# FeggieBoss/raytracing-course

Measured on AMD Instinct MI355X. Metric: Mray/s (closest-hit queries/s), dragon stand-in 1080p/256 spp, RAY_DEPTH 6, higher is better.
Workload: dtype f32

## Files before the change

### raytracing-course_amd/csrc/device/pt_query.h

```cpp
#pragma once
#include "pt_trace.h"

namespace pt {

#ifndef PT_AUXW
#define PT_AUXW 4
#endif

#define PT_LEAF_MARGIN 64.f

PT_HD float h16(uint32_t bits) { return (float)__builtin_bit_cast(_Float16, (uint16_t)(bits & 0xffffu)); }

PT_HD void aux_slab16(uint32_t w0, uint32_t w1, uint32_t w2, f3 inv, f3 oinv, float& tn, float& tf) {
    const float ax = fmaf(h16(w0), inv.x, -oinv.x), bx = fmaf(h16(w1 >> 16), inv.x, -oinv.x);
    const float ay = fmaf(h16(w0 >> 16), inv.y, -oinv.y), by = fmaf(h16(w2), inv.y, -oinv.y);
    const float az = fmaf(h16(w1), inv.z, -oinv.z), bz = fmaf(h16(w2 >> 16), inv.z, -oinv.z);
    tn = fmaxf(fmaxf(fminf(ax, bx), fminf(ay, by)), fminf(az, bz));
    tf = fminf(fminf(fmaxf(ax, bx), fmaxf(ay, by)), fmaxf(az, bz));
}

PT_HD bool aux_entry_hit(const F4& ea, const F4& eb, const Ray& ray, f3 inv, f3 oinv, float dlw) {
    if (signbit(dlw))
        return aux_box_par(h16(f2u(ea.x)), h16(f2u(ea.x) >> 16), h16(f2u(ea.y)), h16(f2u(ea.y) >> 16),
                           h16(f2u(ea.z)), h16(f2u(ea.z) >> 16), ray, inv, oinv);
    float tn, tf, un, uf;
    aux_slab16(f2u(ea.x), f2u(ea.y), f2u(ea.z), inv, oinv, tn, tf);
    aux_slab16(f2u(ea.w), f2u(eb.x), f2u(eb.y), inv, oinv, un, uf);
    const float mt = PT_LEAF_MARGIN * dlw;
    return tn <= tf && tf >= 0.f && (!(mt < INFINITY) || (un - mt <= uf + mt && uf + mt >= 0.f));
}

struct AuxSL { F4 a, b; };
#define PT_AUX_INTERNAL 0xffffffffu

enum : uint32_t { Q_AUX = 0u, Q_REPLAY = 1u, Q_DONE = 2u, Q_EXACT = 3u, Q_DECIDE = 4u };
enum : uint32_t { R_CAND = 0u, R_WALK_E = 1u, R_WALK_N = 2u };
#define PT_RKINDS 3u

#define PT_QPRIM_BYTES 64u
#define PT_QP_FULL 0x100u

PT_HD Prim qprim_expand(const F4& r0, const F4& r1, const F4& r2) {
    Prim P;
    const uint32_t type = f2u(r0.w);
    if (type == T_TRIANGLE) {
        P.p0 = F4{0.f, 0.f, 0.f, r0.w};
        P.p1 = F4{0.f, 0.f, 0.f, 1.f};
        P.p2 = F4{r0.x, r0.y, r0.z, 0.f};
        P.p3 = F4{r1.x, r1.y, r1.z, r2.x};
        P.p4 = F4{r2.y, r2.z, 0.f, 0.f};
    } else {
        P.p0 = F4{r1.x, r1.y, r1.z, r0.w};
        P.p1 = F4{r1.w, r2.x, r2.y, r2.z};
        P.p2 = F4{r0.x, r0.y, r0.z, 0.f};
        P.p3 = F4{0.f, 0.f, 0.f, 0.f};
        P.p4 = F4{0.f, 0.f, 0.f, 0.f};
    }
    return P;
}

#define PT_BUNDLE_BYTES 96u
#define PT_LEAFQ 0x80000000u

#ifndef PT_QHK
#define PT_QHK 6
#endif

struct Query {
    Ray ray;
    f3 inv;
    float P;
    uint32_t phase : 3;
    uint32_t walk : 2;
    uint32_t par : 1;
    uint32_t robust : 1;
    uint32_t known : 1;
    uint32_t overflow : 1;
    uint32_t sp : 7;
    uint32_t pos : 7;
    uint32_t len : 7;
    uint32_t nh : 4;
    uint32_t ne : 4;
    uint32_t cid : 10;
    uint32_t spare : 13;
    uint32_t node;
    uint32_t lb;
    uint32_t cand;
    float dl;
    union {
        struct {
            uint32_t lref, lcnt;
            uint32_t li;
            float lt;
            int lid;
            float lacc;
        };
        struct {
            uint32_t off;
            uint32_t e[4];
            uint32_t astar;
            float bound;
            float t1c, mc;
        };
    };
    uint32_t hidx[PT_QHK];
    float ht[PT_QHK];
    int hid[PT_QHK];
    float hacc[PT_QHK];
    float bt;
    float res_t;
    int res_id;
};
static_assert(PT_QHK < 16, "nh and ne are 4-bit fields");
#define PT_QUERY_SP_MAX 127u

struct QCounts {
    uint32_t nodes, aux, ptests, planes;
#ifdef PT_QDIAG
    uint32_t cands, passes, steps, rc_acc, rc_rej, rc_walk;
#endif
};

struct PlanesGlobal {
    const SceneView& S;
    PT_HD Prim operator()(uint32_t k, uint32_t& pi) const { pi = S.planes[k]; return S.prims[pi]; }
};
template <class PL>
PT_HD void q_planes_e(const SceneView& S, const PL& pl, const Ray& ray, float& P, int& pid) {
    P = PT_INF;
    pid = -1;
    for (uint32_t k = 0; k < S.n_planes; ++k) {
        uint32_t pi;
        const Prim pr = pl(k, pi);
        Hit h;
        bool ok;
        if (f2u(pr.p1.x) == 0u && f2u(pr.p1.y) == 0u && f2u(pr.p1.z) == 0u && f2u(pr.p1.w) == 0x3f800000u) {
            Ray lr;
            lr.o = ray.o + -1.f * mk3(pr.p0.x, pr.p0.y, pr.p0.z);
            lr.d = ray.d;
            ok = isect_plane(lr, mk3(pr.p2.x, pr.p2.y, pr.p2.z), h);
        } else {
            ok = plane_intersect(pr, ray, h);
        }
        if (ok && h.t < P) { P = h.t; pid = (int)pi; }
    }
}
PT_HD void q_planes(const SceneView& S, const Ray& ray, float& P, int& pid) { q_planes_e(S, PlanesGlobal{S}, ray, P, pid); }

PT_HD F4 q_prep(const SceneView& S, const Ray& ray) {
    const float big = 3e38f;
    if (!(fabsf(ray.o.x) < big && fabsf(ray.o.y) < big && fabsf(ray.o.z) < big && fabsf(ray.d.x) < big &&
          fabsf(ray.d.y) < big && fabsf(ray.d.z) < big))
        return F4{0.f, 0.f, 0.f, __builtin_nanf("")};
    const bool par = !replay_ok_ray(ray);
    const float om = fmaxf(fmaxf(fabsf(ray.o.x), fabsf(ray.o.y)), fabsf(ray.o.z));
    const float dm = fminf(fminf(fabsf(ray.d.x), fabsf(ray.d.y)), fabsf(ray.d.z));
    const float dl = par ? -INFINITY : 0x1p-18f * (S.box_extent + om) / dm;
    return F4{1.f / ray.d.x, 1.f / ray.d.y, 1.f / ray.d.z, dl};
}

PT_HD void q_init_pre(const Ray& ray, float P, int pid, F4 pre, Query& q) {
    q.ray = ray;
    q.res_id = pid;
    q.res_t = P;
    q.P = P;
    q.bt = PT_INF;
    q.nh = 0;
    q.ne = 0;
    q.lb = 0;
    q.overflow = 0;
    q.node = 0;
    q.sp = 0;
    q.li = 0;
#pragma unroll
    for (int i = 0; i < PT_QHK; ++i) q.hidx[i] = 0xffffffffu;
    q.inv = mk3(pre.x, pre.y, pre.z);
    q.par = signbit(pre.w) ? 1u : 0u;
    q.dl = fabsf(pre.w);
    q.phase = pre.w != pre.w ? Q_EXACT : Q_AUX;
}

PT_HD void q_init(const SceneView& S, const Ray& ray, float P, int pid, Query& q) {
    q_init_pre(ray, P, pid, q_prep(S, ray), q);
}

template <class T>
PT_HD T q_sel(const T (&a)[PT_QHK], uint32_t k, T dflt) {
    T v = dflt;
#pragma unroll
    for (int i = 0; i < PT_QHK; ++i)
        if ((uint32_t)i == k) v = a[i];
    return v;
}

PT_HD bool q_add_hit(Query& q, uint32_t c, float t, int id, float acc) {
    if (q.ne == PT_QHK) return false;
#pragma unroll
    for (int k = 0; k < PT_QHK; ++k) {
        const bool sw = q.hidx[k] > c;
        const uint32_t xi = q.hidx[k];
        const float xt = q.ht[k];
        const int xd = q.hid[k];
        const float xa = q.hacc[k];
        if (sw) {
            q.hidx[k] = c; q.ht[k] = t; q.hid[k] = id; q.hacc[k] = acc;
            c = xi; t = xt; id = xd; acc = xa;
        }
    }
    if (c != 0xffffffffu) q.overflow = 1u;
    else q.nh = q.nh + 1u;
    return true;
}

PT_HD void q_pass_done(Query& q) {
    if (q.overflow) {
        if (q.ne == PT_QHK) {
            q.phase = Q_EXACT;
            return;
        }
        q.overflow = 0;
        q.node = 0;
        q.sp = 0;
        q.li = 0;
        q.phase = Q_AUX;
        return;
    }
    q.phase = Q_DONE;
}

PT_HD void q_record_entered(Query& q) {
    const float t = q_sel(q.ht, q.ne, PT_INF);
    const int id = q_sel(q.hid, q.ne, -1);
    if (t < q.bt) {
        q.bt = t;
        if (t < q.P) { q.res_t = t; q.res_id = id; }
    }
    q.ne = q.ne + 1u;
    q.lb = q.cand + 1u;
}

PT_HD void q_next_decision(Query& q) { q.phase = Q_DECIDE; }

PT_HD void q_entered(Query& q) {
    q_record_entered(q);
    q_next_decision(q);
}

PT_HD void q_decide(Query& q) {
#pragma unroll 1
    while (q.ne < q.nh) {
        q.cand = q_sel(q.hidx, q.ne, 0xffffffffu);
        if (!(fminf(q.P, q.bt) >= q_sel(q.hacc, q.ne, PT_INF))) {
            q.walk = R_CAND;
            q.phase = Q_REPLAY;
            return;
        }
        q_record_entered(q);
    }
    q_pass_done(q);
}

PT_HD void q_rejected(Query& q) {
#pragma unroll
    for (int k = 0; k + 1 < PT_QHK; ++k) {
        if ((uint32_t)k >= q.ne) {
            q.hidx[k] = q.hidx[k + 1];
            q.ht[k] = q.ht[k + 1];
            q.hid[k] = q.hid[k + 1];
            q.hacc[k] = q.hacc[k + 1];
        }
    }
    q.hidx[PT_QHK - 1] = 0xffffffffu;
    q.nh = q.nh - 1u;
    q.lb = q.cand + 1u;
    q_next_decision(q);
}

PT_HD float q_bound_between(const Query& q, uint32_t a, uint32_t r) {
    float m = q.P;
    bool any = false;
#pragma unroll
    for (int k = 0; k < PT_QHK; ++k) {
        if ((uint32_t)k < q.ne && q.hidx[k] > a && q.hidx[k] < r) {
            if (!any || q.ht[k] < m) m = q.ht[k];
            any = true;
        }
    }
    return m;
}

PT_HD float q_leaf_accept_t(const Query& q, const F4& na, const F4& nb) {
    const f3 c = mk3(na.x, na.y, na.z);
    const f3 s = mk3(na.w, nb.x, nb.y);
    const f3 o = q.ray.o + -1.f * c;
    const f3 nlo = -1.f * s - o, nhi = s - o;
    const float ax = nlo.x * q.inv.x, bx = nhi.x * q.inv.x;
    const float ay = nlo.y * q.inv.y, by = nhi.y * q.inv.y;
    const float az = nlo.z * q.inv.z, bz = nhi.z * q.inv.z;
    const float t1 = smax(smax(smin(ax, bx), smin(ay, by)), smin(az, bz));
    const float t2 = smin(smin(smax(ax, bx), smax(ay, by)), smax(az, bz));
    const float m = q.dl + (fabsf(t1) + fabsf(t2)) * 0x1p-18f;
    const bool robust = !q.par && t1 + m <= t2 - m && t2 - m >= 0.f;
    return robust ? t1 + m : INFINITY;
}

PT_HD uint32_t q_leaf_certain(Query& q, const Node& nd) {
    float lo = q.P, hi = q.P;
#pragma unroll
    for (int k = 0; k < PT_QHK; ++k)
        if ((uint32_t)k < q.ne) { lo = fminf(lo, q.ht[k]); hi = fmaxf(hi, q.ht[k]); }
    const f3 c = mk3(nd.a.x, nd.a.y, nd.a.z);
    const f3 s = mk3(nd.a.w, nd.b.x, nd.b.y);
    const f3 o = q.ray.o + -1.f * c;
    const f3 nlo = -1.f * s - o, nhi = s - o;
    const float ax = nlo.x * q.inv.x, bx = nhi.x * q.inv.x;
    const float ay = nlo.y * q.inv.y, by = nhi.y * q.inv.y;
    const float az = nlo.z * q.inv.z, bz = nhi.z * q.inv.z;
    const float t1 = smax(smax(smin(ax, bx), smin(ay, by)), smin(az, bz));
    const float t2 = smin(smin(smax(ax, bx), smax(ay, by)), smax(az, bz));
    const float m = q.dl + (fabsf(t1) + fabsf(t2)) * 0x1p-18f;
    q.t1c = t1;
    q.mc = m;
    q.robust = (!q.par && t1 + m <= t2 - m && t2 - m >= 0.f) ? 1u : 0u;
    if (q.robust && lo >= t1 + m) return 1u;
    uint32_t v = q.par ? 2u : enter_decide(t1, t2, hi);
    if (v == 2u) v = enter_exact(nd.a, nd.b, q.ray, hi) ? 1u : 0u;
    return v == 0u ? 0u : 2u;
}


PT_HD void q_addr(const SceneView& S, const Query& q, uint32_t off[8]) {
    uint32_t b0, b1, b2;
    if (q.phase == Q_AUX) {
        if (!(q.node & PT_LEAFQ)) {
            const uint32_t b = S.o_aux + q.node * (uint32_t)(PT_AUXW * sizeof(AuxSL));
#pragma unroll
            for (int k = 0; k < 8; ++k) off[k] = b + 16u * (uint32_t)k;
            return;
        }
        if (q.li == 0u) {
            b0 = S.o_bundle + PT_BUNDLE_BYTES * (q.node & 0x7fffffffu);
#pragma unroll
            for (int k = 0; k < 8; ++k) off[k] = b0 + 16u * (uint32_t)(k < 6 ? k : 5);
            return;
        }
        if (q.li & 0x80000000u) {
            b0 = S.o_prim + 80u * (q.lref + (q.li & 0x7fffffffu));
#pragma unroll
            for (int k = 0; k < 8; ++k) off[k] = b0 + 16u * (uint32_t)(k < 5 ? k : 4);
            return;
        }
        b0 = S.o_qprim + PT_QPRIM_BYTES * (q.lref + q.li);
#pragma unroll
        for (int k = 0; k < 8; ++k) off[k] = b0 + 16u * (uint32_t)(k < 4 ? k : 3);
        return;
    } else if (q.walk == R_CAND) {
        b0 = S.o_nodes + 32u * q.cand;
        b1 = b0 + 16u;
        b2 = S.o_ainfo + 16u * (q.cand >> 2);
    } else if (q.walk == R_WALK_E) {
        b0 = S.o_anc + 4u * (q.off + q.pos);
        b1 = b0;
        b2 = b0;
    } else {
#pragma unroll
        for (int j = 0; j < 4; ++j) {
            const uint32_t e = q.e[j] == 0xffffffffu ? 0u : q.e[j];
            off[2 * j] = S.o_nodes + 32u * e;
            off[2 * j + 1] = off[2 * j] + 16u;
        }
        return;
    }
    off[0] = b0; off[1] = b1; off[2] = b2;
#pragma unroll
    for (int k = 3; k < 8; ++k) off[k] = b0;
}

template <class Mem>
PT_HD void q_aux_next(Query& q, Mem& stk, uint32_t next) {
    if (next == 0xffffffffu && q.sp > 0u) next = stk.get(--q.sp);
    if (next != 0xffffffffu) {
        q.node = next;
        return;
    }
    q_next_decision(q);
}

#if defined(PT_QPROF) && defined(__HIP_DEVICE_COMPILE__)
#define PT_QPROF_DEV 1
#define QP_STAMP(i) do { uint64_t t_; asm volatile("s_memtime %0\n\ts_waitcnt lgkmcnt(0)" : "=s"(t_)::"memory"); qp[i] = (uint32_t)t_; } while (0)
#define QP_ARG , uint32_t* qp
#else
#define QP_STAMP(i) (void)0
#define QP_ARG
#endif
template <class Mem>
PT_HD void q_exec_aux(const SceneView& S, Query& q, QCounts& C, Mem& stk, const F4 r[8]) {
    C.aux++;
    const f3 oinv = mk3(q.ray.o.x * q.inv.x, q.ray.o.y * q.inv.y, q.ray.o.z * q.inv.z);
    const float mt = PT_LEAF_MARGIN * q.dl;
    const bool mwide = !(mt < INFINITY);
    bool hit[PT_AUXW];
#pragma unroll
    for (int k = 0; k < PT_AUXW; ++k) {
        const F4 ea = r[2 * k], eb = r[2 * k + 1];
        float tn, tf, un, uf;
        aux_slab16(f2u(ea.x), f2u(ea.y), f2u(ea.z), q.inv, oinv, tn, tf);
        aux_slab16(f2u(ea.w), f2u(eb.x), f2u(eb.y), q.inv, oinv, un, uf);
        hit[k] = tn <= tf && tf >= 0.f && (mwide || (un - mt <= uf + mt && uf + mt >= 0.f));
    }
    if (pt_any(q.par != 0u)) {
#pragma unroll
        for (int k = 0; k < PT_AUXW; ++k) {
            const F4 ea = r[2 * k];
            if (q.par)
                hit[k] = aux_box_par(h16(f2u(ea.x)), h16(f2u(ea.x) >> 16), h16(f2u(ea.y)), h16(f2u(ea.y) >> 16),
                                     h16(f2u(ea.z)), h16(f2u(ea.z) >> 16), q.ray, q.inv, oinv);
        }
    }
    uint32_t next = 0xffffffffu;
    const uint32_t hmax = q.hidx[PT_QHK - 1];
    uint32_t sp = q.sp;
    bool ovf = false;
#pragma unroll
    for (int k = 0; k < PT_AUXW; ++k) {
        const uint32_t code = f2u(r[2 * k + 1].w);
        const uint32_t rng = f2u(r[2 * k + 1].z);
        const bool h = hit[k] && code != 0xffffffffu;
        const bool isleaf = (code & 0x80000000u) != 0u;
        const uint32_t lidx = code & 0x7fffffffu;
        const bool above = isleaf ? lidx > hmax
                                  : (hmax != 0xffffffffu && ((rng & 0xffffu) << S.aux_rshift) > hmax);
        const bool fresh = isleaf ? lidx >= q.lb : ((rng >> 16) << S.aux_rshift) >= q.lb;
        ovf = ovf || (h && fresh && above);
        const bool take = h && fresh && !above;
        const uint32_t item = isleaf ? (PT_LEAFQ | rng) : code;
        const bool first = take && next == 0xffffffffu;
        const bool push = take && !first;
        next = first ? item : next;
        stk.setc(sp, item, push && sp < stk.cap);
        sp += push ? 1u : 0u;
    }
    if (ovf) q.overflow = 1u;
    if (sp > stk.cap) {
        q.phase = Q_EXACT;
        return;
    }
    q.sp = sp;
#ifdef PT_QDIAG
    if (next == 0xffffffffu && q.sp == 0u) C.passes++;
    if (q.sp > C.steps) C.steps = q.sp;
#endif
    q_aux_next(q, stk, next);
}

template <class Mem>
PT_HD void q_exec_kind(const SceneView& S, Query& q, QCounts& C, Mem& stk, const F4 r[8] QP_ARG) {
    if (q.phase == Q_AUX && !(q.node & PT_LEAFQ)) {
        QP_STAMP(0);
        q_exec_aux(S, q, C, stk, r);
        return;
    }
    if (q.phase == Q_AUX) {
        QP_STAMP(1);
        if (q.li == 0u) {
            q.cand = f2u(r[3].x);
            q.lref = f2u(r[3].y);
            q.lcnt = f2u(r[3].z);
            q.lt = PT_INF;
            q.lid = -1;
            q.lacc = q_leaf_accept_t(q, r[4], r[5]);
#ifdef PT_QDIAG
            C.cands++;
#endif
            if (q.lcnt == 0u) {
                q_aux_next(q, stk, 0xffffffffu);
                return;
            }
        }
        const bool full = (q.li & 0x80000000u) != 0u;
        const uint32_t cty = f2u(r[0].w);
        if (!full && (cty & PT_QP_FULL)) {
            q.li |= 0x80000000u;
            return;
        }
        Prim pr = qprim_expand(r[0], r[1], r[2]);
        if (full) { pr.p0 = r[0]; pr.p1 = r[1]; pr.p2 = r[2]; pr.p3 = r[3]; pr.p4 = r[4]; }
        const uint32_t ty = f2u(pr.p0.w);
        Ray lr = q.ray;
        if (full || cty != T_TRIANGLE) {
            const f3 pos = mk3(pr.p0.x, pr.p0.y, pr.p0.z);
            lr.o = q.ray.o + -1.f * pos;
            const bool ident = f2u(pr.p1.x) == 0u && f2u(pr.p1.y) == 0u && f2u(pr.p1.z) == 0u &&
                               f2u(pr.p1.w) == 0x3f800000u;
            if (!ident) {
                q4 qq;
                qq.x = pr.p1.x; qq.y = pr.p1.y; qq.z = pr.p1.z; qq.w = pr.p1.w;
                const q4 cq = conj(qq);
                lr.o = qrot(cq, lr.o);
                lr.d = qrot(cq, q.ray.d);
            }
        }
        const f3 pa = mk3(pr.p2.x, pr.p2.y, pr.p2.z);
        bool ok;
        float t = 0.f;
        uint32_t in;
        if (ty == T_TRIANGLE) {
            const f3 pb = mk3(pr.p3.x, pr.p3.y, pr.p3.z), pc = mk3(pr.p3.w, pr.p4.x, pr.p4.y);
            f3 n = mk3(r[1].w, r[2].w, q.li == 0u ? r[3].w : r[3].x);
            if (full) n = normalize(cross(pb - pa, pc - pa));
            Hit h;
            ok = isect_triangle_n(lr, pa, pb, pc, n, h);
            t = h.t;
        } else if (ty == T_BOX) {
            ok = slab(lr.o, lr.d, pa, t, in);
        } else {
            ok = ellipsoid_root(lr, pa, t, in);
        }
        const uint32_t li = q.li & 0x7fffffffu;
        C.ptests++;
        if (ok && t < q.lt) { q.lt = t; q.lid = (int)(q.lref + li); }
        q.li = li + 1u;
        if (q.li < q.lcnt) return;
        q.li = 0u;
        if (q.lid >= 0 && !q_add_hit(q, q.cand, q.lt, q.lid, q.lacc)) {
            q.phase = Q_EXACT;
            return;
        }
        q_aux_next(q, stk, 0xffffffffu);
        return;
    }
    if (q.walk == R_CAND) {
        QP_STAMP(2);
        Node nd;
        nd.a = r[0];
        nd.b = r[1];
        const uint32_t k4 = q.cand & 3u;
        const uint32_t info = f2u(k4 == 0u ? r[2].x : k4 == 1u ? r[2].y : k4 == 2u ? r[2].z : r[2].w);
        C.nodes++;
        const uint32_t v = q_leaf_certain(q, nd);
#ifdef PT_QDIAG
        if (v == 1u) C.rc_acc++; else if (v == 0u) C.rc_rej++; else C.rc_walk++;
#endif
        if (v == 1u) {
            q_entered(q);
            return;
        }
        if (v == 0u) {
            q_rejected(q);
            return;
        }
        q.off = info & 0x03ffffffu;
        q.len = info >> 26;
        q.pos = 0u;
        q.known = q.ne == 0u ? 1u : 0u;
        q.bound = q.P;
        q.astar = 0u;
        q.walk = R_WALK_E;
        return;
    }
    if (q.walk == R_WALK_E) {
        QP_STAMP(3);
        const uint32_t hlast = q_sel(q.hidx, q.ne - 1u, 0u);
        bool any = false, accept = false;
        const uint32_t ent[4] = {f2u(r[0].x), f2u(r[0].y), f2u(r[0].z), f2u(r[0].w)};
#pragma unroll
        for (int j = 0; j < 4; ++j) {
            uint32_t e = q.pos + (uint32_t)j < q.len ? ent[j] : 0xffffffffu;
            if (e != 0xffffffffu && !accept && !q.known) {
                if (e <= hlast) {
                    q.astar = e;
                    e = 0xffffffffu;
                } else {
                    q.bound = q_bound_between(q, q.astar, e);
                    q.known = 1u;
                    if (q.robust && q.bound >= q.t1c + q.mc) accept = true;
                }
            }
            if (accept) e = 0xffffffffu;
            q.e[j] = e;
            any = any || e != 0xffffffffu;
        }
        if (accept) {
            q_entered(q);
            return;
        }
        if (any) q.walk = R_WALK_N;
        else q.pos += 4u;
        return;
    }
    QP_STAMP(4);
    bool reject = false;
#pragma unroll
    for (int j = 0; j < 4; ++j) {
        if (q.e[j] == 0xffffffffu) continue;
        Node nd;
        nd.a = r[2 * j];
        nd.b = r[2 * j + 1];
        C.nodes++;
        if (!node_enter(nd, q.ray, q.inv, q.bound, q.par != 0u)) reject = true;
    }
    if (reject) {
        q_rejected(q);
        return;
    }
    q.pos += 4u;
    if (q.pos >= q.len) q_entered(q);
    else q.walk = R_WALK_E;
}

template <class Mem>
PT_HD void q_exec(const SceneView& S, Query& q, QCounts& C, Mem& stk, const F4 r[8] QP_ARG) {
#ifdef PT_QPROF_DEV
    q_exec_kind(S, q, C, stk, r, qp);
#else
    q_exec_kind(S, q, C, stk, r);
#endif
    if (q.phase == Q_DECIDE) q_decide(q);
}

PT_HD F4 blob_piece(const SceneView& S, uint32_t off) {
    return *reinterpret_cast<const F4*>(reinterpret_cast<const unsigned char*>(S.blob) + off);
}

template <class Mem>
PT_HD void q_step(const SceneView& S, Query& q, QCounts& C, Mem& stk) {
    uint32_t off[8];
    q_addr(S, q, off);
    F4 r[8];
#pragma unroll
    for (int k = 0; k < 8; ++k) r[k] = blob_piece(S, off[k]);
#ifdef PT_QPROF_DEV
    uint32_t qp[5];
    q_exec(S, q, C, stk, r, qp);
#else
    q_exec(S, q, C, stk, r);
#endif
}

template <class Mem>
PT_HD void q_aux_step(const SceneView& S, Query& q, QCounts& C, Mem& stk) {
    const uint32_t b = S.o_aux + q.node * (uint32_t)(PT_AUXW * sizeof(AuxSL));
    F4 r[8];
#pragma unroll
    for (int k = 0; k < 8; ++k) r[k] = blob_piece(S, b + 16u * (uint32_t)k);
    q_exec_aux(S, q, C, stk, r);
    if (q.phase == Q_DECIDE) q_decide(q);
}

template <class Stack>
PT_HD int q_exact(const SceneView& S, const Ray& ray, Stack& stk, Hit& out, QCounts& C) {
    SceneView E = S;
    E.aux = nullptr;
    Counts X{};
    const ReplayCfg cfg{0u, 0u};
    const int id = ray_intersection<false>(E, cfg, ray, stk, out, X);
    C.nodes += (uint32_t)X.nodes;
    C.ptests += (uint32_t)X.ptests;
    C.planes += (uint32_t)X.planes;
    return id;
}

template <class Stack>
PT_HD int q_run(const SceneView& S, const Ray& ray, Stack& stk, Hit& out, QCounts& C, uint32_t& exact_used) {
    Query q;
    float P;
    int pid;
    q_planes(S, ray, P, pid);
    C.planes += S.n_planes;
    q_init(S, ray, P, pid, q);
    while (q.phase == Q_AUX || q.phase == Q_REPLAY) q_step(S, q, C, stk);
    exact_used = q.phase == Q_EXACT ? 1u : 0u;
    if (exact_used) return q_exact(S, ray, stk, out, C);
    if (q.res_id >= 0) {
        const bool ok = prim_intersect(S.prims[q.res_id], ray, out);
        if (!ok || f2u(out.t) != f2u(q.res_t)) C.planes |= 0x80000000u;
    }
    return q.res_id;
}

}
```

Before: 4994.

## Defer hit-list edits to wave-uniform blocks after query step dispatch

Hit-list insertion and rejection no longer happen inside the divergent per-phase branches. Each branch records the edit in a small QEdit record, and q_exec applies it afterward in blocks guarded by pt_any, so lanes doing the same edit share one code path. The insertion sort is rewritten as a branchless shift with selects, and the aux-node range tests are simplified into shared lo/hi bounds combined with bitwise ops. The aim is less divergence and fewer duplicated register-heavy sort copies. The cost is an extra struct carried through the step, and edits are now applied after q_aux_next and q_next_decision rather than before them, which reorders state updates.

```diff
diff --git a/raytracing-course_amd/csrc/device/pt_query.h b/raytracing-course_amd/csrc/device/pt_query.h
--- a/raytracing-course_amd/csrc/device/pt_query.h
+++ b/raytracing-course_amd/csrc/device/pt_query.h
@@ -193,23 +193,28 @@
     return v;
 }
 
-PT_HD bool q_add_hit(Query& q, uint32_t c, float t, int id, float acc) {
-    if (q.ne == PT_QHK) return false;
-#pragma unroll
-    for (int k = 0; k < PT_QHK; ++k) {
-        const bool sw = q.hidx[k] > c;
-        const uint32_t xi = q.hidx[k];
-        const float xt = q.ht[k];
-        const int xd = q.hid[k];
-        const float xa = q.hacc[k];
-        if (sw) {
-            q.hidx[k] = c; q.ht[k] = t; q.hid[k] = id; q.hacc[k] = acc;
-            c = xi; t = xt; id = xd; acc = xa;
-        }
-    }
-    if (c != 0xffffffffu) q.overflow = 1u;
+enum : uint32_t { QE_NONE = 0u, QE_ADD = 1u, QE_REJECT = 2u };
+struct QEdit {
+    uint32_t op;
+    uint32_t c;
+    float t;
+    int id;
+    float acc;
+};
+
+PT_HD void q_add_hit(Query& q, uint32_t c, float t, int id, float acc) {
+    if (q.hidx[PT_QHK - 1] != 0xffffffffu) q.overflow = 1u;
     else q.nh = q.nh + 1u;
-    return true;
+#pragma unroll
+    for (int k = PT_QHK - 1; k >= 0; --k) {
+        const int l = k > 0 ? k - 1 : 0;
+        const bool up = q.hidx[k] > c;
+        const bool upl = k > 0 && q.hidx[l] > c;
+        q.ht[k] = up ? (upl ? q.ht[l] : t) : q.ht[k];
+        q.hid[k] = up ? (upl ? q.hid[l] : id) : q.hid[k];
+        q.hacc[k] = up ? (upl ? q.hacc[l] : acc) : q.hacc[k];
+        q.hidx[k] = up ? (upl ? q.hidx[l] : c) : q.hidx[k];
+    }
 }
 
 PT_HD void q_pass_done(Query& q) {
@@ -260,7 +265,12 @@
     q_pass_done(q);
 }
 
-PT_HD void q_rejected(Query& q) {
+PT_HD void q_rejected(Query& q, QEdit& ed) {
+    ed.op = QE_REJECT;
+    q.lb = q.cand + 1u;
+    q_next_decision(q);
+}
+PT_HD void q_drop_rejected(Query& q) {
 #pragma unroll
     for (int k = 0; k + 1 < PT_QHK; ++k) {
         if ((uint32_t)k >= q.ne) {
@@ -272,8 +282,6 @@
     }
     q.hidx[PT_QHK - 1] = 0xffffffffu;
     q.nh = q.nh - 1u;
-    q.lb = q.cand + 1u;
-    q_next_decision(q);
 }
 
 PT_HD float q_bound_between(const Query& q, uint32_t a, uint32_t r) {
@@ -407,7 +415,7 @@
         float tn, tf, un, uf;
         aux_slab16(f2u(ea.x), f2u(ea.y), f2u(ea.z), q.inv, oinv, tn, tf);
         aux_slab16(f2u(ea.w), f2u(eb.x), f2u(eb.y), q.inv, oinv, un, uf);
-        hit[k] = tn <= tf && tf >= 0.f && (mwide || (un - mt <= uf + mt && uf + mt >= 0.f));
+        hit[k] = (tn <= tf) & (tf >= 0.f) & (mwide | ((un - mt <= uf + mt) & (uf + mt >= 0.f)));
     }
     if (pt_any(q.par != 0u)) {
 #pragma unroll
@@ -429,9 +437,10 @@
         const bool h = hit[k] && code != 0xffffffffu;
         const bool isleaf = (code & 0x80000000u) != 0u;
         const uint32_t lidx = code & 0x7fffffffu;
-        const bool above = isleaf ? lidx > hmax
-                                  : (hmax != 0xffffffffu && ((rng & 0xffffu) << S.aux_rshift) > hmax);
-        const bool fresh = isleaf ? lidx >= q.lb : ((rng >> 16) << S.aux_rshift) >= q.lb;
+        const uint32_t rlo = isleaf ? lidx : (rng & 0xffffu) << S.aux_rshift;
+        const uint32_t rhi = isleaf ? lidx : (rng >> 16) << S.aux_rshift;
+        const bool above = rlo > hmax;
+        const bool fresh = rhi >= q.lb;
         ovf = ovf || (h && fresh && above);
         const bool take = h && fresh && !above;
         const uint32_t item = isleaf ? (PT_LEAFQ | rng) : code;
@@ -455,7 +464,7 @@
 }
 
 template <class Mem>
-PT_HD void q_exec_kind(const SceneView& S, Query& q, QCounts& C, Mem& stk, const F4 r[8] QP_ARG) {
+PT_HD void q_exec_kind(const SceneView& S, Query& q, QCounts& C, Mem& stk, const F4 r[8], QEdit& ed QP_ARG) {
     if (q.phase == Q_AUX && !(q.node & PT_LEAFQ)) {
         QP_STAMP(0);
         q_exec_aux(S, q, C, stk, r);
@@ -523,9 +532,12 @@
         q.li = li + 1u;
         if (q.li < q.lcnt) return;
         q.li = 0u;
-        if (q.lid >= 0 && !q_add_hit(q, q.cand, q.lt, q.lid, q.lacc)) {
-            q.phase = Q_EXACT;
-            return;
+        if (q.lid >= 0) {
+            if (q.ne == PT_QHK) {
+                q.phase = Q_EXACT;
+                return;
+            }
+            ed = QEdit{QE_ADD, q.cand, q.lt, q.lid, q.lacc};
         }
         q_aux_next(q, stk, 0xffffffffu);
         return;
@@ -547,7 +559,7 @@
             return;
         }
         if (v == 0u) {
-            q_rejected(q);
+            q_rejected(q, ed);
             return;
         }
         q.off = info & 0x03ffffffu;
@@ -601,7 +613,7 @@
         if (!node_enter(nd, q.ray, q.inv, q.bound, q.par != 0u)) reject = true;
     }
     if (reject) {
-        q_rejected(q);
+        q_rejected(q, ed);
         return;
     }
     q.pos += 4u;
@@ -611,11 +623,18 @@
 
 template <class Mem>
 PT_HD void q_exec(const SceneView& S, Query& q, QCounts& C, Mem& stk, const F4 r[8] QP_ARG) {
+    QEdit ed{QE_NONE, 0u, 0.f, 0, 0.f};
 #ifdef PT_QPROF_DEV
-    q_exec_kind(S, q, C, stk, r, qp);
+    q_exec_kind(S, q, C, stk, r, ed, qp);
 #else
-    q_exec_kind(S, q, C, stk, r);
-#endif
+    q_exec_kind(S, q, C, stk, r, ed);
+#endif
+    if (pt_any(ed.op == QE_ADD)) {
+        if (ed.op == QE_ADD) q_add_hit(q, ed.c, ed.t, ed.id, ed.acc);
+    }
+    if (pt_any(ed.op == QE_REJECT)) {
+        if (ed.op == QE_REJECT) q_drop_rejected(q);
+    }
     if (q.phase == Q_DECIDE) q_decide(q);
 }
 
```

Result: faster. 5387, median of 6 (+7.9%).
